# lattice/quda

Hardware: NVIDIA H100
Metric: wilson_dslash_gflops (higher is better)
Workload: dtype f32

## Files before the change

quda_b200/csrc/clover.h:

```cpp
#pragma once

#include "core.h"

namespace b200
{

  template <class P> struct CloverView {
    using store = typename P::store;
    const store *c[2];
    int volume_cb;
    int compressed;
    int dynamic;
    typename P::real diagonal;
    float nrm;
  };

  template <class P> struct CholT { using type = double; };
  template <> struct CholT<PrecH16> { using type = float; };

  template <class P, int CB> B2_HD void clover_load_block(typename P::real *a, const CloverView<P> &A, int x_cb, int parity, int chi)
  {
    using real = typename P::real;
    using V = typename P::svec;
    constexpr int N = P::Ns;
    constexpr int M = (CB + N - 1) / N;
    constexpr int Moff = CB / N;
    real tmp[M * N];
    const V *base = reinterpret_cast<const V *>(A.c[parity]);
#pragma unroll
    for (int i = 0; i < M; i++) {
      const V w = ld<Cache::STREAM>(base + (size_t)(chi * Moff + i) * A.volume_cb + x_cb);
      vec_to_real(tmp + i * N, w);
      if constexpr (P::fixed) {
#pragma unroll
        for (int j = 0; j < N; j++) tmp[i * N + j] *= A.nrm;
      }
    }
    const int sh = (chi * CB) % N;
    if constexpr (CB == 36) {
#pragma unroll
      for (int i = 0; i < 36; i++) a[i] = tmp[i + sh];
    } else {
#pragma unroll
      for (int i = 0; i < 4; i++) a[i] = tmp[i + sh];
#pragma unroll
      for (int i = 6; i < 30; i++) a[i] = tmp[i - 2 + sh];
#pragma unroll
      for (int i = 0; i < 3; i++) {
        const real dev = a[i];
        a[i + 3] = A.diagonal - dev;
        a[i] = A.diagonal + dev;
      }
      a[30] = -a[6];
      a[31] = -a[7];
      a[32] = -a[8];
      a[33] = -a[9];
      a[34] = -a[16];
      a[35] = -a[17];
    }
  }

  B2_HD constexpr int tri_idx(int i, int j) { return 6 + 2 * (15 - (6 - j) * (5 - j) / 2 + i - j - 1); }

  template <typename real> B2_HD void hmat_mul(real *y, const real *a, const real *x)
  {
#pragma unroll
    for (int i = 0; i < 6; i++) {
      real re = a[i] * x[2 * i], im = a[i] * x[2 * i + 1];
#pragma unroll
      for (int j = 0; j < 6; j++) {
        if (j == i) continue;
        const int k = (j < i) ? tri_idx(i, j) : tri_idx(j, i);
        const real ar = a[k];
        const real ai = (j < i) ? a[k + 1] : -a[k + 1];
        re += ar * x[2 * j];
        re -= ai * x[2 * j + 1];
        im += ar * x[2 * j + 1];
        im += ai * x[2 * j];
      }
      y[2 * i] = re;
      y[2 * i + 1] = im;
    }
  }

  template <typename T, typename real> B2_HD void hmat_solve(real *x, const real *a)
  {
    T Lr[6][6], Li[6][6];
#pragma unroll
    for (int i = 0; i < 6; i++) {
#pragma unroll
      for (int j = 0; j < 6; j++) {
        if (j > i) continue;
        T sr = 0, si = 0;
#pragma unroll
        for (int k = 0; k < 6; k++) {
          if (k >= j) continue;
          sr += Lr[i][k] * Lr[j][k];
          sr += Li[i][k] * Li[j][k];
          si += Li[i][k] * Lr[j][k];
          si -= Lr[i][k] * Li[j][k];
        }
        if (i == j) {
          const T d = (T)a[i] - sr;
#if defined(__CUDA_ARCH__)
          Lr[i][i] = (sizeof(T) == 8) ? (T)::rsqrt((double)d) : (T)::rsqrtf((float)d);
#else
          Lr[i][i] = (T)1 / std::sqrt(d);
#endif
          Li[i][i] = 0;
        } else {
          const int k = tri_idx(i, j);
          Lr[i][j] = ((T)a[k] - sr) * Lr[j][j];
          Li[i][j] = ((T)a[k + 1] - si) * Lr[j][j];
        }
      }
    }
    T yr[6], yi[6];
#pragma unroll
    for (int i = 0; i < 6; i++) {
      T r = x[2 * i], m = x[2 * i + 1];
#pragma unroll
      for (int j = 0; j < 6; j++) {
        if (j >= i) continue;
        r -= Lr[i][j] * yr[j];
        r += Li[i][j] * yi[j];
        m -= Lr[i][j] * yi[j];
        m -= Li[i][j] * yr[j];
      }
      yr[i] = r * Lr[i][i];
      yi[i] = m * Lr[i][i];
    }
#pragma unroll
    for (int i = 5; i >= 0; i--) {
      T r = yr[i], m = yi[i];
#pragma unroll
      for (int j = 0; j < 6; j++) {
        if (j <= i) continue;
        r -= Lr[j][i] * yr[j];
        r -= Li[j][i] * yi[j];
        m -= Lr[j][i] * yi[j];
        m += Li[j][i] * yr[j];
      }
      yr[i] = r * Lr[i][i];
      yi[i] = m * Lr[i][i];
    }
#pragma unroll
    for (int i = 0; i < 6; i++) {
      x[2 * i] = (real)yr[i];
      x[2 * i + 1] = (real)yi[i];
    }
  }

  template <class P, bool inverse> B2_HD void clover_apply_site(typename P::real *v, const CloverView<P> &A, int x_cb, int parity)
  {
    using real = typename P::real;
    real r[24];
#pragma unroll
    for (int c = 0; c < 3; c++) {
#pragma unroll
      for (int z = 0; z < 2; z++) {
        const real v0 = v[(0 * 3 + c) * 2 + z], v1 = v[(1 * 3 + c) * 2 + z];
        const real v2 = v[(2 * 3 + c) * 2 + z], v3 = v[(3 * 3 + c) * 2 + z];
        r[(0 * 3 + c) * 2 + z] = -v1 - v3;
        r[(1 * 3 + c) * 2 + z] = v2 + v0;
        r[(2 * 3 + c) * 2 + z] = v3 - v1;
        r[(3 * 3 + c) * 2 + z] = v0 - v2;
      }
    }
#pragma unroll
    for (int chi = 0; chi < 2; chi++) {
      real a[36];
      if (A.compressed)
        clover_load_block<P, 28>(a, A, x_cb, parity, chi);
      else
        clover_load_block<P, 36>(a, A, x_cb, parity, chi);
      if (inverse && A.dynamic) {
        hmat_solve<typename CholT<P>::type>(r + 12 * chi, a);
#pragma unroll
        for (int i = 0; i < 12; i++) r[12 * chi + i] *= (real)0.25;
      } else {
        real y[12];
        hmat_mul(y, a, r + 12 * chi);
#pragma unroll
        for (int i = 0; i < 12; i++) r[12 * chi + i] = y[i];
      }
    }
#pragma unroll
    for (int c = 0; c < 3; c++) {
#pragma unroll
      for (int z = 0; z < 2; z++) {
        const real r0 = r[(0 * 3 + c) * 2 + z], r1 = r[(1 * 3 + c) * 2 + z];
        const real r2 = r[(2 * 3 + c) * 2 + z], r3 = r[(3 * 3 + c) * 2 + z];
        v[(0 * 3 + c) * 2 + z] = r1 + r3;
        v[(1 * 3 + c) * 2 + z] = -r2 - r0;
        v[(2 * 3 + c) * 2 + z] = -r3 + r1;
        v[(3 * 3 + c) * 2 + z] = -r0 + r2;
      }
    }
  }

}
```

quda_b200/csrc/core.h:

```cpp
#pragma once

#include <cmath>
#include <cstddef>
#include <cstdint>
#include <cstring>
#include <type_traits>
#include <utility>

#if defined(__CUDACC__)
#define B2_HD __host__ __device__ __forceinline__
#define B2_D __device__ __forceinline__
#else
#define B2_HD inline
#define B2_D inline
#endif

namespace b200
{

  struct alignas(16) f4 { float x, y, z, w; };
  struct alignas(16) d2 { double x, y; };
  struct alignas(8) f2 { float x, y; };
  struct alignas(16) s8 { short v[8]; };
  struct alignas(8) s4 { short v[4]; };
// ... 371 lines not shown
      }
#pragma unroll
      for (int i = 0; i < 24 / N; i++) {
        V o;
        store *e = reinterpret_cast<store *>(&o);
#pragma unroll
        for (int j = 0; j < N; j++) {
          if constexpr (P::fixed)
            e[j] = f2s(t[i * N + j]);
          else
            e[j] = t[i * N + j];
        }
        st_stream(base + (size_t)i * stride + x_cb, o);
      }
    }
  };

  template <class P> struct GhostView {
    using store = typename P::store;
    store *v;
    float *norm;
    int face_cb;

    B2_HD void load(typename P::real *out, int idx) const
    {
      using V = typename P::ghost_vec;
      constexpr int N = P::Ng;
      const V *base = reinterpret_cast<const V *>(v);
#pragma unroll
      for (int i = 0; i < 12 / N; i++) {
        const V t = ld<Cache::COHERENT>(base + (size_t)i * face_cb + idx);
        vec_to_real(out + i * N, t);
      }
      if constexpr (P::fixed) {
        const float n = ld<Cache::COHERENT>(norm + idx);
#pragma unroll
        for (int i = 0; i < 12; i++) out[i] *= n;
      }
    }

    B2_HD void save(const typename P::real *in, int idx) const
    {
      using V = typename P::ghost_vec;
      constexpr int N = P::Ng;
      V *base = reinterpret_cast<V *>(v);
      typename P::real t[12];
#pragma unroll
      for (int i = 0; i < 12; i++) t[i] = in[i];
      if constexpr (P::fixed) {
        float mx = 0.0f;
#pragma unroll
        for (int i = 0; i < 12; i++) mx = fmaxf(mx, fabsf(t[i]));
        norm[idx] = mx * kFixedInvMax;
        const float sinv = fast_div(kFixedMax, mx);
#pragma unroll
        for (int i = 0; i < 12; i++) t[i] *= sinv;
      }
#pragma unroll
      for (int i = 0; i < 12 / N; i++) {
        V o;
        store *e = reinterpret_cast<store *>(&o);
#pragma unroll
        for (int j = 0; j < N; j++) {
          if constexpr (P::fixed)
            e[j] = f2s(t[i * N + j]);
          else
            e[j] = t[i * N + j];
        }
        base[(size_t)i * face_cb + idx] = o;
      }
    }
  };

  struct GaugeMeta {
    double anisotropy;
    double link_max;
    int t_boundary;
    int first_time_slice;
    int last_time_slice;
    int t_bound_cb;
    int volume_cb;
  };

  template <class P, int recon> struct GaugeView {
    using real = typename P::real;
    using store = typename P::store;
    using V = typename GaugeVec<P, recon>::vec;
    static constexpr int N = GaugeVec<P, recon>::N;
    static constexpr int M = recon / N;

    const store *g[2];
    int stride;
    real aniso, tb, link_scale;
    int t_bound_cb, volume_cb, first_ts, last_ts;

    B2_HD void init(const void *base, size_t parity_offset_bytes, int stride_, const GaugeMeta &m)
    {
      g[0] = reinterpret_cast<const store *>(base);
      g[1] = reinterpret_cast<const store *>(reinterpret_cast<const char *>(base) + parity_offset_bytes);
      stride = stride_;
      aniso = (real)m.anisotropy;
      tb = (real)m.t_boundary;
      link_scale = (real)m.link_max;
      t_bound_cb = m.t_bound_cb;
      volume_cb = m.volume_cb;
      first_ts = m.first_time_slice;
      last_ts = m.last_time_slice;
    }

    B2_HD real u0(int dir, int idx) const
    {
      if (dir < 3) return aniso;
      if (idx >= volume_cb) return first_ts ? tb : (real)1;
      if (idx >= t_bound_cb) return last_ts ? tb : (real)1;
      return (real)1;
    }

    struct Raw {
      V w[M];
    };

    template <Cache c = Cache::STREAM> B2_HD void load_raw(Raw &r, int dir, int x_cb, int parity) const
    {
      const V *base = reinterpret_cast<const V *>(g[parity]);
#pragma unroll
      for (int i = 0; i < M; i++) r.w[i] = ld<c>(base + (size_t)(dir * M + i) * stride + x_cb);
    }

    B2_HD void unpack(real *u, const Raw &r, int dir, int x_cb) const
    {
      real t[recon];
#pragma unroll
      for (int i = 0; i < M; i++) {
        vec_to_real(t + i * N, r.w[i]);
        if constexpr (P::fixed) {
#pragma unroll
          for (int j = 0; j < N; j++) t[i * N + j] *= kFixedInvMax;
        }
      }
      if constexpr (recon == 18) {
#pragma unroll
        for (int i = 0; i < 18; i++) u[i] = P::fixed ? link_scale * t[i] : t[i];
      } else if constexpr (recon == 12) {
#pragma unroll
        for (int i = 0; i < 12; i++) u[i] = t[i];
        const real s = u0(dir, x_cb);
        const cplx<real> a0 {u[0], u[1]}, a1 {u[2], u[3]}, a2 {u[4], u[5]};
        const cplx<real> b0 {u[6], u[7]}, b1 {u[8], u[9]}, b2 {u[10], u[11]};
        cplx<real> c0 = cmul(a1, b2), c1 = cmul(a2, b0), c2 = cmul(a0, b1);
        const cplx<real> d0 = cmul(a2, b1), d1 = cmul(a0, b2), d2_ = cmul(a1, b0);
        u[12] = s * (c0.re - d0.re);
        u[13] = -s * (c0.im - d0.im);
        u[14] = s * (c1.re - d1.re);
        u[15] = -s * (c1.im - d1.im);
        u[16] = s * (c2.re - d2_.re);
        u[17] = -s * (c2.im - d2_.im);
      } else {
        unpack8(u, t, u0(dir, x_cb));
      }
    }

    B2_HD void unpack_deferred(real *u, real &scale, const Raw &r, int dir, int x_cb) const
    {
      static_assert(P::fixed, "deferred scaling is for the fixed-point formats");
      if constexpr (recon == 8) {
        unpack(u, r, dir, x_cb);
        scale = (real)1;
      } else {
        real t[recon];
        vecs_to_real<M, N>(t, r.w);
        if constexpr (recon == 18) {
#pragma unroll
          for (int i = 0; i < 18; i++) u[i] = t[i];
          scale = link_scale * kFixedInvMax;
        } else {
#pragma unroll
          for (int i = 0; i < 12; i++) u[i] = t[i];
          const real s = u0(dir, x_cb) * kFixedInvMax;
          const cplx<real> a0 {u[0], u[1]}, a1 {u[2], u[3]}, a2 {u[4], u[5]};
          const cplx<real> b0 {u[6], u[7]}, b1 {u[8], u[9]}, b2 {u[10], u[11]};
          cplx<real> c0 = cmul(a1, b2), c1 = cmul(a2, b0), c2 = cmul(a0, b1);
          const cplx<real> d0 = cmul(a2, b1), d1 = cmul(a0, b2), d2_ = cmul(a1, b0);
          u[12] = s * (c0.re - d0.re);
          u[13] = -s * (c0.im - d0.im);
          u[14] = s * (c1.re - d1.re);
          u[15] = -s * (c1.im - d1.im);
          u[16] = s * (c2.re - d2_.re);
          u[17] = -s * (c2.im - d2_.im);
          scale = kFixedInvMax;
        }
      }
    }

    template <Cache c = Cache::STREAM> B2_HD void load(real *u, int dir, int x_cb, int parity) const
    {
      Raw r;
      load_raw<c>(r, dir, x_cb, parity);
      unpack(u, r, dir, x_cb);
    }

    B2_HD static void unpack8(real *u, const real *in, real u0v)
    {
      const real u0_inv = rcp_((real)u0v);
      cplx<real> o[9];
      o[1] = {in[2], in[3]};
      o[2] = {in[4], in[5]};
      o[3] = {in[6], in[7]};
      real sn, cs;
      sincospi_(in[0], &sn, &cs);
      o[0] = {cs, sn};
      sincospi_(in[1], &sn, &cs);
      o[6] = {cs, sn};
      real row_sum = mul_rn(o[1].re, o[1].re);
      row_sum = fma_rn(o[1].im, o[1].im, row_sum);
      row_sum = fma_rn(o[2].re, o[2].re, row_sum);
      row_sum = fma_rn(o[2].im, o[2].im, row_sum);
      const real row_sum_inv = rcp_(row_sum);
      real diff = fma_rn(u0_inv, u0_inv, -row_sum);
      const real m00 = diff > 0 ? diff * rsqrt_(diff) : (real)0;
      o[0].re *= m00;
      o[0].im *= m00;
      real col_sum = mul_rn(o[0].re, o[0].re);
      col_sum = fma_rn(o[0].im, o[0].im, col_sum);
      col_sum = fma_rn(o[3].re, o[3].re, col_sum);
      col_sum = fma_rn(o[3].im, o[3].im, col_sum);
      diff = fma_rn(u0_inv, u0_inv, -col_sum);
      const real m20 = diff > 0 ? diff * rsqrt_(diff) : (real)0;
      o[6].re *= m20;
      o[6].im *= m20;
      const real r_inv2 = u0_inv * row_sum_inv;
      {
        cplx<real> A = cmul(conj(o[0]), o[3]);
        A.re *= u0v;
        A.im *= u0v;
        cplx<real> t4 = cmul(conj(o[6]), conj(o[2]));
        const cplx<real> a1 = cmul(A, o[1]);
        o[4] = {-r_inv2 * (t4.re + a1.re), -r_inv2 * (t4.im + a1.im)};
        cplx<real> t5 = cmul(conj(o[6]), conj(o[1]));
        const cplx<real> a2 = cmul(A, o[2]);
        o[5] = {r_inv2 * (t5.re - a2.re), r_inv2 * (t5.im - a2.im)};
      }
      {
        cplx<real> A = cmul(conj(o[0]), o[6]);
        A.re *= u0v;
        A.im *= u0v;
        cplx<real> t7 = cmul(conj(o[3]), conj(o[2]));
        const cplx<real> a1 = cmul(A, o[1]);
        o[7] = {r_inv2 * (t7.re - a1.re), r_inv2 * (t7.im - a1.im)};
        cplx<real> t8 = cmul(conj(o[3]), conj(o[1]));
        const cplx<real> a2 = cmul(A, o[2]);
        o[8] = {-r_inv2 * (t8.re + a2.re), -r_inv2 * (t8.im + a2.im)};
      }
#pragma unroll
      for (int i = 0; i < 3; i++) {
        u[2 * i] = o[i + 3].re;
        u[2 * i + 1] = o[i + 3].im;
        u[6 + 2 * i] = o[i].re;
        u[6 + 2 * i + 1] = o[i].im;
        u[12 + 2 * i] = -o[i + 6].re;
        u[12 + 2 * i + 1] = -o[i + 6].im;
      }
    }

    B2_HD static float rcp_(float x)
    {
#if defined(__CUDA_ARCH__)
      return __frcp_rn(x);
#else
      return 1.0f / x;
#endif
    }
    B2_HD static double rcp_(double x) { return 1.0 / x; }
    B2_HD static void sincospi_(float x, float *s, float *c)
    {
#if defined(__CUDA_ARCH__)
      __sincosf(x * 3.14159265358979323846f, s, c);
#else
      *s = (float)std::sin(3.14159265358979323846 * (double)x);
      *c = (float)std::cos(3.14159265358979323846 * (double)x);
#endif
    }
    B2_HD static void sincospi_(double x, double *s, double *c)
    {
#if defined(__CUDA_ARCH__)
      ::sincospi(x, s, c);
#else
      *s = std::sin(3.14159265358979323846 * x);
      *c = std::cos(3.14159265358979323846 * x);
#endif
    }
    B2_HD static float rsqrt_(float x)
    {
#if defined(__CUDA_ARCH__)
      return ::rsqrtf(x);
#else
      return 1.0f / std::sqrt(x);
#endif
    }
    B2_HD static double rsqrt_(double x)
    {
#if defined(__CUDA_ARCH__)
      return ::rsqrt(x);
#else
      return 1.0 / std::sqrt(x);
#endif
    }
  };

  template <bool adjoint, typename real> B2_HD void su3_mul(real *r, const real *u, const real *h)
  {
#pragma unroll
    for (int s = 0; s < 2; s++) {
#pragma unroll
      for (int i = 0; i < 3; i++) {
        real re = 0, im = 0;
#pragma unroll
        for (int j = 0; j < 3; j++) {
          const real ur = adjoint ? u[(j * 3 + i) * 2] : u[(i * 3 + j) * 2];
          const real ui = adjoint ? -u[(j * 3 + i) * 2 + 1] : u[(i * 3 + j) * 2 + 1];
          const real hr = h[(s * 3 + j) * 2], hi = h[(s * 3 + j) * 2 + 1];
          re = fma_rn(ur, hr, re);
          re = fma_rn(-ui, hi, re);
          im = fma_rn(ur, hi, im);
          im = fma_rn(ui, hr, im);
        }
        r[(s * 3 + i) * 2] = re;
        r[(s * 3 + i) * 2 + 1] = im;
      }
    }
  }

  template <typename real> B2_HD void project(real *h, const real *v, int mu, int sign)
  {
    const real sg = (real)sign;
#pragma unroll
    for (int c = 0; c < 3; c++) {
      const real v0r = v[(0 * 3 + c) * 2], v0i = v[(0 * 3 + c) * 2 + 1];
      const real v1r = v[(1 * 3 + c) * 2], v1i = v[(1 * 3 + c) * 2 + 1];
      const real v2r = v[(2 * 3 + c) * 2], v2i = v[(2 * 3 + c) * 2 + 1];
      const real v3r = v[(3 * 3 + c) * 2], v3i = v[(3 * 3 + c) * 2 + 1];
      real h0r, h0i, h1r, h1i;
      if (mu == 0) {
        h0r = v0r - sg * v3i;
        h0i = v0i + sg * v3r;
        h1r = v1r - sg * v2i;
        h1i = v1i + sg * v2r;
      } else if (mu == 1) {
        h0r = v0r + sg * v3r;
        h0i = v0i + sg * v3i;
        h1r = v1r - sg * v2r;
        h1i = v1i - sg * v2i;
      } else if (mu == 2) {
        h0r = v0r - sg * v2i;
        h0i = v0i + sg * v2r;
        h1r = v1r + sg * v3i;
// ... 83 lines not shown
```

quda_b200/csrc/kernels.cuh:

```cuda
#pragma once

#include <cstdlib>
#include <cuda_runtime.h>

#include "dslash_site.h"
#include "plan.h"

namespace b200
{

#ifndef B2_MINBLOCKS_F64
#define B2_MINBLOCKS_F64 2
#endif
#ifndef B2_MINBLOCKS_F32
#define B2_MINBLOCKS_F32 4
#endif
#ifndef B2_MINBLOCKS_H16
#define B2_MINBLOCKS_H16 4
#endif
  template <class P> struct MinBlocks { static constexpr int value = B2_MINBLOCKS_F32; };
  template <> struct MinBlocks<PrecF64> { static constexpr int value = B2_MINBLOCKS_F64; };
  template <> struct MinBlocks<PrecH16> { static constexpr int value = B2_MINBLOCKS_H16; };

#ifndef B2_L2_PREFETCH
#define B2_L2_PREFETCH 0
#endif
  __device__ __forceinline__ void prefetch_l2(const void *p) { asm volatile("prefetch.global.L2 [%0];" ::"l"(p)); }

  template <class P, int recon>
  __device__ __forceinline__ void prefetch_future_tile(const DslashArgs<P, recon> &arg, const TileMap &tm)
  {
    using GV = GaugeView<P, recon>;
    constexpr int lanes_per_line = 128 / sizeof(typename GV::V);
    if ((threadIdx.x & ((1 << tm.sh[0]) - 1)) % lanes_per_line != 0) return;
    const unsigned gx = gridDim.x, gy = gridDim.y, gz = gridDim.z;
    unsigned lin = blockIdx.x + gx * (blockIdx.y + gy * blockIdx.z) + B2_L2_PREFETCH;
    if (lin >= gx * gy * gz) return;
    const unsigned bz = lin / (gx * gy);
    lin -= bz * gx * gy;
    const unsigned by = lin / gx;
    const unsigned bx = lin - by * gx;
    int x[4], x_cb, parity;
    if (!tile_site(x, x_cb, parity, arg.geom, tm, arg.n_parity, arg.parity, bx, by, bz, threadIdx.x)) return;
    const Geom &g = arg.geom;
    const typename GV::V *gf = reinterpret_cast<const typename GV::V *>(arg.U.g[parity]);
    const typename GV::V *gb = reinterpret_cast<const typename GV::V *>(arg.U.g[1 - parity]);
#pragma unroll
    for (int d = 0; d < 4; d++) {
      int y[4] = {x[0], x[1], x[2], x[3]};
      y[d] = (x[d] - 1 < 0) ? g.X[d] - 1 : x[d] - 1;
      const int n_cb = cb_from_coords(y, g);
#pragma unroll
      for (int i = 0; i < GV::M; i++) {
        prefetch_l2(gf + (size_t)(d * GV::M + i) * arg.U.stride + x_cb);
        prefetch_l2(gb + (size_t)(d * GV::M + i) * arg.U.stride + n_cb);
      }
    }
  }

  template <class P, int recon, bool dagger, bool xpay, OpType op, bool part>
  __global__ void __launch_bounds__(kMaxTile, MinBlocks<P>::value)
    dslash_interior_kernel(const __grid_constant__ DslashArgs<P, recon> arg, const __grid_constant__ TileMap tm)
  {
    if constexpr (B2_L2_PREFETCH > 0) prefetch_future_tile(arg, tm);
    int x[4], x_cb, parity;
    if (!tile_site(x, x_cb, parity, arg.geom, tm, arg.n_parity, arg.parity, blockIdx.x, blockIdx.y, blockIdx.z, threadIdx.x))
      return;
    dslash_site_interior<P, recon, dagger, xpay, op, part>(arg, x, x_cb, parity);
  }

  __device__ __forceinline__ unsigned ld_acquire_sys(const unsigned *p)
  {
    unsigned v;
    asm volatile("ld.acquire.sys.global.u32 %0, [%1];" : "=r"(v) : "l"(p) : "memory");
    return v;
  }
  __device__ __forceinline__ void st_release_sys(unsigned *p, unsigned v)
  {
    asm volatile("st.release.sys.global.u32 [%0], %1;" ::"l"(p), "r"(v) : "memory");
  }
  __device__ __forceinline__ void red_release_sys_add(unsigned *p, unsigned v)
  {
    asm volatile("red.release.sys.global.add.u32 [%0], %1;" ::"l"(p), "r"(v) : "memory");
  }

  template <class Arg> __device__ __forceinline__ void wait_for_halo(const Arg &arg)
  {
    if (threadIdx.x == 0) {
      const long long t0 = clock64();
      const unsigned uses = (arg.seq + (arg.seq & 1u)) >> 1;
#pragma unroll
      for (int d = 0; d < 4; d++) {
#pragma unroll
        for (int dir = 0; dir < 2; dir++) {
          const unsigned *f = arg.wait_flag[d][dir];
          if (!f) continue;
          const unsigned target = uses * (unsigned)arg.geom.face_cb[d];
          while ((int)(ld_acquire_sys(f) - target) < 0) {
            if (clock64() - t0 > 20000000000LL) {
              if (arg.timeout_flag) *arg.timeout_flag = 1;
              break;
            }
            __nanosleep(100);
          }
        }
      }
    }
    __syncthreads();
  }

  template <class P, int recon, bool dagger, bool xpay, OpType op>
  __global__ void __launch_bounds__(kMaxTile, MinBlocks<P>::value)
    dslash_boundary_kernel(const __grid_constant__ DslashArgs<P, recon> arg, const __grid_constant__ TileMap tm,
                           const __grid_constant__ SlabTable st)
  {
    wait_for_halo(arg);
    const int parity = arg.n_parity == 2 ? blockIdx.y : arg.parity;
    int x[4], x_cb;
    if (!slab_site(x, x_cb, arg.geom, tm, st, parity, blockIdx.x, threadIdx.x)) return;
    dslash_site_full<P, recon, dagger, xpay, op>(arg, x, x_cb, parity);
  }

  template <class P, int recon, bool dagger, bool xpay, OpType op>
  __global__ void __launch_bounds__(256) dslash_exterior_kernel(const __grid_constant__ DslashArgs<P, recon> arg)
  {
    wait_for_halo(arg);
    const int parity = arg.n_parity == 2 ? blockIdx.y : arg.parity;
    const int tid = blockIdx.x * blockDim.x + threadIdx.x;
    if (tid >= arg.threads_ext[4]) return;
    int x[4], x_cb;
    if (!exterior_thread_site(x, x_cb, arg, tid, parity)) return;
    dslash_site_exterior<P, recon, dagger, xpay, op>(arg, x, x_cb, parity);
  }

  template <class P, bool inverse>
  __global__ void __launch_bounds__(256) clover_apply_kernel(SpinorView<P> out, SpinorView<P> in, CloverView<P> A,
                                                             int volume_cb, int parity)
  {
    const int x_cb = blockIdx.x * blockDim.x + threadIdx.x;
    if (x_cb >= volume_cb) return;
    typename P::real v[24];
    in.template load<Cache::COHERENT>(v, x_cb);
    clover_apply_site<P, inverse>(v, A, x_cb, parity);
    out.save(v, x_cb);
  }

// ... 244 lines not shown
    count_launch();
    return check_cuda(cudaGetLastError(), "copy_gauge launch");
  }

  template <class P> int launch_gauge_copy_precision(const GaugeCopyRequest &rq)
  {
    const bool dbl = rq.host_precision == 8;
    switch (rq.native.reconstruct) {
    case 18: return dbl ? launch_gauge_copy_typed<P, 18, double>(rq) : launch_gauge_copy_typed<P, 18, float>(rq);
    case 12: return dbl ? launch_gauge_copy_typed<P, 12, double>(rq) : launch_gauge_copy_typed<P, 12, float>(rq);
    case 8: return dbl ? launch_gauge_copy_typed<P, 8, double>(rq) : launch_gauge_copy_typed<P, 8, float>(rq);
    }
    return set_error(B200_ERR_INVALID, "reconstruct %d not in {18,12,8}", rq.native.reconstruct);
  }

  template <class P, typename H>
  __global__ void __launch_bounds__(128) copy_clover_kernel(typename P::store *c0, typename P::store *c1, const H *packed,
                                                            int volume_cb, int compressed, double diagonal, double nrm_inv)
  {
    using store = typename P::store;
    constexpr int N = P::Ns;
    const int x = blockIdx.x * blockDim.x + threadIdx.x;
    if (x >= volume_cb) return;
    const int parity = blockIdx.y;
    store *dst = parity ? c1 : c0;
    const H *src = packed + ((size_t)parity * volume_cb + x) * 72;
    const int CB = compressed ? 28 : 36;
#pragma unroll
    for (int chi = 0; chi < 2; chi++) {
      double a[36];
#pragma unroll
      for (int i = 0; i < 36; i++) a[i] = 0.5 * (double)src[chi * 36 + i];
      for (int k = 0; k < CB; k++) {
        double v;
        if (!compressed)
          v = a[k];
        else if (k < 3)
          v = a[k] - diagonal;
        else if (k == 3)
          v = 0.0;
        else
          v = a[k + 2];
        const int flat = chi * CB + k;
        store o;
        if constexpr (P::fixed)
          o = f2s((float)(v * nrm_inv));
        else
          o = (store)v;
        dst[((size_t)(flat / N) * volume_cb + x) * N + flat % N] = o;
      }
    }
  }

  template <class P> int launch_clover_copy_precision(const CloverCopyRequest &rq)
  {
    Geom g;
    geom_init(g, rq.X);
    auto *c0 = reinterpret_cast<typename P::store *>(const_cast<void *>(rq.native.clover));
    auto *c1 = reinterpret_cast<typename P::store *>(reinterpret_cast<char *>(const_cast<void *>(rq.native.clover)) + rq.native.parity_stride_bytes);
    const double nrm_inv = P::fixed ? (2.0 * 32767.0) / rq.native.max_element : 1.0;
    dim3 grid((g.volume_cb + 127) / 128, 2, 1);
    cudaStream_t s = (cudaStream_t)rq.stream;
    if (rq.host_precision == 8)
      copy_clover_kernel<P, double><<<grid, 128, 0, s>>>(c0, c1, (const double *)rq.packed, g.volume_cb, rq.native.compressed, rq.native.diagonal, nrm_inv);
    else
      copy_clover_kernel<P, float><<<grid, 128, 0, s>>>(c0, c1, (const float *)rq.packed, g.volume_cb, rq.native.compressed, rq.native.diagonal, nrm_inv);
    count_launch();
    return check_cuda(cudaGetLastError(), "copy_clover launch");
  }

  template <class P, int recon, bool dagger, bool xpay, OpType op>
  int launch_config(OpCfg<dagger, xpay, op>, const LaunchRequest &rq, const DslashArgs<P, recon> &arg)
  {
    LaunchPlan pl;
    if (int rc = plan_dslash(pl, rq, arg)) return rc;
    cudaStream_t s = (cudaStream_t)rq.stream;
    for (int i = 0; i < pl.n; i++) {
      const LaunchStep &l = pl.step[i];
      const dim3 grid(l.grid[0], l.grid[1], l.grid[2]);
      switch (l.kind) {
      case LAUNCH_INTERIOR:
        if (l.masked)
          dslash_interior_kernel<P, recon, dagger, xpay, op, true><<<grid, l.threads, 0, s>>>(arg, l.tm);
        else
          dslash_interior_kernel<P, recon, dagger, xpay, op, false><<<grid, l.threads, 0, s>>>(arg, l.tm);
        break;
      case LAUNCH_BOUNDARY: dslash_boundary_kernel<P, recon, dagger, xpay, op><<<grid, l.threads, 0, s>>>(arg, l.tm, l.st); break;
      case LAUNCH_EXTERIOR: dslash_exterior_kernel<P, recon, dagger, xpay, op><<<grid, l.threads, 0, s>>>(arg); break;
      case LAUNCH_FUSED: {
        PackArgs<P> pk {};
        if (rq.fused_pack) fill_pack_args(pk, *rq.fused_pack);
        dslash_fused_kernel<P, recon, dagger, xpay, op><<<grid, l.threads, 0, s>>>(arg, l.tm, pk, l.fs);
        break;
      }
      }
      count_launch();
    }
    return check_cuda(cudaGetLastError(), rq.fused_pack ? "fused dslash launch" : "dslash launch");
  }

  template <class P> int launch_precision(const LaunchRequest &rq)
  {
    return dispatch_dslash<P>(rq, [&](auto c, const auto &arg) { return launch_config(c, rq, arg); });
  }

  template <class P> int launch_clover_precision(const CloverRequest &rq)
  {
    SpinorView<P> out, in;
    CloverView<P> A;
    fill_spinor(out, rq.out, rq.out_norm, rq.volume_cb);
    fill_spinor(in, rq.in, rq.in_norm, rq.volume_cb);
    fill_clover(A, rq.A, rq.volume_cb);
    const int blocks = (rq.volume_cb + 127) / 128;
    cudaStream_t s = (cudaStream_t)rq.stream;
    if (rq.inverse)
      clover_apply_kernel<P, true><<<blocks, 128, 0, s>>>(out, in, A, rq.volume_cb, rq.parity);
    else
      clover_apply_kernel<P, false><<<blocks, 128, 0, s>>>(out, in, A, rq.volume_cb, rq.parity);
    count_launch();
    return check_cuda(cudaGetLastError(), "clover launch");
  }

  template <class P> int launch_twist_precision(const TwistRequest &rq)
  {
    SpinorView<P> out, in;
    fill_spinor(out, rq.out, rq.out_norm, rq.volume_cb);
    fill_spinor(in, rq.in, rq.in_norm, rq.volume_cb);
    twist_gamma5_kernel<P><<<(rq.volume_cb + 255) / 256, 256, 0, (cudaStream_t)rq.stream>>>(out, in, rq.volume_cb, (typename P::real)rq.a,
                                                                                          (typename P::real)rq.b);
    count_launch();
    return check_cuda(cudaGetLastError(), "twist launch");
  }

  template <class P> int launch_pack_precision(const PackRequest &rq)
  {
    int gx;
    if (int rc = pack_blocks(gx, rq)) return rc;
    if (!gx) return 0;
    PackArgs<P> arg;
    fill_pack_args(arg, rq);
    pack_kernel<P><<<dim3(gx, 8, 1), 128, 0, (cudaStream_t)rq.stream>>>(arg);
    count_launch();
    return check_cuda(cudaGetLastError(), "pack launch");
  }

  template <class P> int launch_pack_multi_precision(const PackRequest &rq, const PackBatchRequest &b)
  {
    int gx;
    if (int rc = pack_blocks(gx, rq)) return rc;
    if (!gx) return 0;
    PackArgs<P> arg;
    fill_pack_args(arg, rq);
    PackBatch<P> batch;
    fill_pack_batch(batch, b, arg.geom.volume_cb);
    pack_multi_kernel<P><<<dim3(gx, 8, b.n_src), 128, 0, (cudaStream_t)rq.stream>>>(arg, batch);
    count_launch();
    return check_cuda(cudaGetLastError(), "batched pack launch");
  }

}
```

quda_b200/csrc/launch.h:

```cpp
#pragma once

#include <cstdarg>
#include <cstdio>
#include <cuda_runtime.h>

#include "../../include/b200_dslash.h"
#include "dslash_site.h"

namespace b200
{

  int set_error(int code, const char *fmt, ...);
  int check_cuda(cudaError_t e, const char *what);
  void count_launch();

  struct LaunchRequest {
    int op, kernel, reconstruct, dagger, xpay, parity, n_parity;
    int X[4], tile[4];
    double b;
    int asymmetric;
    int tma;
    int tma_ty, tma_tz, tma_grid;
    int tma_link_slots;
    int tma_center_slots, tma_halo_slots;
// ... 39 lines not shown
    int volume_cb, host_precision, to_native;
    void *stream;
  };

  struct GaugeCopyRequest {
    b200_gauge native;
    int X[4];
    void *qdp[4], *ghost[4];
    int host_precision;
    void *stream;
  };

  struct CloverCopyRequest {
    b200_clover native;
    int X[4];
    const void *packed;
    int host_precision;
    void *stream;
  };

  struct PackRequest {
    int X[4], parity, dagger, comm_dim[4];
    void *in, *in_norm;
    void *dst[4][2], *dst_norm[4][2];
    void *signal[4][2];
    int *block_counter;
    unsigned seq;
    void *stream;
  };

  inline size_t ghost_parity_bytes(int precision, const int X[4], int dim)
  {
    const size_t face_cb = (size_t)X[0] * X[1] * X[2] * X[3] / X[dim] / 2;
    return face_cb * (12 * (size_t)precision + (precision == B200_HALF ? 4 : 0));
  }

  inline int check_src_stride(const char *what, int n_src, int precision, const int X[4], const int comm_dim[4], const size_t stride[4],
                              int n_parity)
  {
    for (int d = 0; d < 4; d++) {
      if (!comm_dim[d] || n_src <= 1) continue;
      const size_t slab = (size_t)n_parity * ghost_parity_bytes(precision, X, d);
      if (stride[d] < slab)
        return set_error(B200_ERR_INVALID, "%s[%d] = %zu is smaller than one face (%zu bytes): every source needs its own ghost slab", what, d,
                         stride[d], slab);
      if (stride[d] % 16) return set_error(B200_ERR_INVALID, "%s[%d] = %zu is not a multiple of 16 bytes", what, d, stride[d]);
    }
    return 0;
  }

  struct PackBatchRequest {
    int n_src;
    void *in[B200_MAX_MULTI_RHS], *in_norm[B200_MAX_MULTI_RHS];
    size_t dst_stride[4];
  };

  template <class P> void fill_spinor(SpinorView<P> &v, void *base, void *norm, int volume_cb)
  {
    v.v = reinterpret_cast<typename P::store *>(base);
    v.stride = volume_cb;
    if (P::fixed)
      v.norm = norm ? reinterpret_cast<float *>(norm) :
                      reinterpret_cast<float *>(reinterpret_cast<short *>(base) + (size_t)24 * volume_cb);
    else
      v.norm = nullptr;
  }

  template <class P> void fill_spinor_parity(SpinorView<P> &v, const b200_spinor &f, int p)
  {
    char *base = reinterpret_cast<char *>(f.v) + (size_t)p * f.parity_stride_bytes;
    char *norm = f.norm ? reinterpret_cast<char *>(f.norm) + (size_t)p * f.parity_stride_bytes : nullptr;
    fill_spinor(v, base, norm, f.volume_cb);
  }

  template <class P> void fill_clover(CloverView<P> &A, const b200_clover &c, int volume_cb)
  {
    A.c[0] = reinterpret_cast<const typename P::store *>(c.clover);
    A.c[1] = reinterpret_cast<const typename P::store *>(reinterpret_cast<const char *>(c.clover) + c.parity_stride_bytes);
    A.volume_cb = volume_cb;
    A.compressed = c.compressed;
    A.dynamic = c.dynamic_inverse;
    A.diagonal = (typename P::real)c.diagonal;
    A.nrm = (float)(c.max_element / (2.0 * 32767.0));
  }

  template <class P> void fill_ghost(GhostView<P> &g, void *base, void *norm, int face_cb)
  {
    g.v = reinterpret_cast<typename P::store *>(base);
    g.face_cb = face_cb;
    if (P::fixed)
      g.norm = norm ? reinterpret_cast<float *>(norm) :
                      (base ? reinterpret_cast<float *>(reinterpret_cast<short *>(base) + (size_t)12 * face_cb) : nullptr);
    else
      g.norm = nullptr;
  }

  template <class P> B2_HD GhostView<P> ghost_of_source(GhostView<P> g, size_t bytes)
  {
    g.v = reinterpret_cast<typename P::store *>(reinterpret_cast<char *>(g.v) + bytes);
    if (g.norm) g.norm = reinterpret_cast<float *>(reinterpret_cast<char *>(g.norm) + bytes);
    return g;
  }

  template <class P, int recon> int fill_args(DslashArgs<P, recon> &arg, const LaunchRequest &rq)
  {
    geom_init(arg.geom, rq.X);
    const Geom &g = arg.geom;
    arg.n_parity = rq.n_parity;
    arg.parity = rq.parity;
    arg.a = (typename P::real)rq.a;
    arg.A = CloverView<P> {};
    arg.A.diagonal = (typename P::real)(rq.dagger ? -rq.b : rq.b);
    if (rq.out.volume_cb != g.volume_cb || rq.in.volume_cb != g.volume_cb)
      return set_error(B200_ERR_INVALID, "spinor volume_cb (%d/%d) does not match lattice (%d)", rq.out.volume_cb,
                       rq.in.volume_cb, g.volume_cb);
    if (rq.n_parity == 2) {
      for (int p = 0; p < 2; p++) {
        fill_spinor_parity(arg.out[p], rq.out, p);
        fill_spinor_parity(arg.in[p], rq.in, p);
        if (rq.xpay) fill_spinor_parity(arg.x[p], rq.x, p);
      }
    } else {
      fill_spinor_parity(arg.out[rq.parity], rq.out, 0);
      fill_spinor_parity(arg.in[1 - rq.parity], rq.in, 0);
      if (rq.xpay) fill_spinor_parity(arg.x[rq.parity], rq.x, 0);
    }
    GaugeMeta m;
    m.anisotropy = rq.U.anisotropy;
    m.link_max = rq.U.link_max;
    m.t_boundary = rq.U.t_boundary;
    m.first_time_slice = rq.U.first_time_slice;
    m.last_time_slice = rq.U.last_time_slice;
    m.t_bound_cb = (g.X[3] - 1) * g.X[0] * g.X[1] * g.X[2] / 2;
    m.volume_cb = g.volume_cb;
    arg.U.init(rq.U.gauge, rq.U.parity_stride_bytes, rq.U.stride, m);
    if (rq.op == OP_CLOVER || rq.op == OP_CLOVER_PC) fill_clover(arg.A, rq.A, g.volume_cb);
    arg.threads_ext[0] = 0;
    for (int d = 0; d < 4; d++) {
      arg.comm_dim[d] = rq.halo.comm_dim[d] ? 1 : 0;
      if (arg.comm_dim[d] && g.X[d] < 4)
        return set_error(B200_ERR_INVALID, "partitioned dimension %d needs local extent >= 4 (got %d)", d, g.X[d]);
      arg.threads_ext[d + 1] = arg.threads_ext[d] + (arg.comm_dim[d] ? 2 * g.face_cb[d] : 0);
      const size_t parity_elems = (size_t)12 * g.face_cb[d] + (P::fixed ? 2 * g.face_cb[d] : 0);
      arg.ghost_parity_stride[d] = rq.n_parity == 2 ? parity_elems : 0;
      arg.ghost_norm_parity_stride[d] = rq.n_parity == 2 ? parity_elems / 2 : 0;
      for (int dir = 0; dir < 2; dir++) {
        if (arg.comm_dim[d] && rq.kernel != B200_KERNEL_INTERIOR && rq.kernel != B200_KERNEL_INTERIOR_TILES
            && rq.kernel != B200_KERNEL_INTERIOR_SITES && !rq.halo.ghost[d][dir])
          return set_error(B200_ERR_INVALID, "dimension %d is partitioned but halo.ghost[%d][%d] is NULL", d, d, dir);
        fill_ghost(arg.ghost[d][dir], rq.halo.ghost[d][dir], rq.halo.ghost_norm[d][dir], g.face_cb[d]);
        arg.wait_flag[d][dir] = arg.comm_dim[d] ? reinterpret_cast<const unsigned *>(rq.halo.wait_flag[d][dir]) : nullptr;
      }
    }
    arg.seq = rq.halo.seq;
    arg.timeout_flag = rq.halo.timeout_flag;
    return 0;
  }


  template <class P> int mrhs_batch(int remaining, int max_batch)
  {
    int cap = sizeof(typename P::real) == 8 ? 2 : 4;
    if (max_batch > 0 && max_batch < cap) cap = max_batch;
    if (remaining >= 4 && cap >= 4) return 4;
    if (remaining >= 2 && cap >= 2) return 2;
    return 1;
// ... 306 lines not shown
```

Baseline: 6387.

## Defer fixed-point clover scaling, specialize float Cholesky, speed recon-8 unpack, add PDL launch

For half-precision clover, the per-element dequantization multiply is dropped and the scale is applied once on output, with a quantized diagonal and inverse scale precomputed on the host. A float specialization of the Cholesky solve uses FMAs and a reciprocal-diagonal array. Recon-8 gauge unpacking for fixed precision folds the pi scale into fast sincos, uses a precomputed inverse anisotropy, and uses an approximate reciprocal with a Newton step. The unmasked interior kernel is now launched with programmatic dependent launch so it can overlap the previous kernel's tail. The fixed-point changes do not apply to f32, and fast sincos and the approximate reciprocal lower accuracy in the half path.

New measurement: 6498 (median of 6 runs). No clear change (+1.7%).

```diff
diff --git a/quda_b200/csrc/clover.h b/quda_b200/csrc/clover.h
--- a/quda_b200/csrc/clover.h
+++ b/quda_b200/csrc/clover.h
@@ -5,7 +5,13 @@
 namespace b200
 {
 
-  template <class P> struct CloverView {
+  template <class P> struct CloverFixedScale {};
+  template <> struct CloverFixedScale<PrecH16> {
+    float diagonal_q;
+    float inv_scale;
+  };
+
+  template <class P> struct CloverView : CloverFixedScale<P> {
     using store = typename P::store;
     const store *c[2];
     int volume_cb;
@@ -31,10 +37,6 @@
     for (int i = 0; i < M; i++) {
       const V w = ld<Cache::STREAM>(base + (size_t)(chi * Moff + i) * A.volume_cb + x_cb);
       vec_to_real(tmp + i * N, w);
-      if constexpr (P::fixed) {
-#pragma unroll
-        for (int j = 0; j < N; j++) tmp[i * N + j] *= A.nrm;
-      }
     }
     const int sh = (chi * CB) % N;
     if constexpr (CB == 36) {
@@ -45,11 +47,16 @@
       for (int i = 0; i < 4; i++) a[i] = tmp[i + sh];
 #pragma unroll
       for (int i = 6; i < 30; i++) a[i] = tmp[i - 2 + sh];
+      real diag;
+      if constexpr (P::fixed)
+        diag = A.diagonal_q;
+      else
+        diag = A.diagonal;
 #pragma unroll
       for (int i = 0; i < 3; i++) {
         const real dev = a[i];
-        a[i + 3] = A.diagonal - dev;
-        a[i] = A.diagonal + dev;
+        a[i + 3] = diag - dev;
+        a[i] = diag + dev;
       }
       a[30] = -a[6];
       a[31] = -a[7];
@@ -151,6 +158,79 @@
     }
   }
 
+  template <> B2_HD void hmat_solve<float, float>(float *x, const float *a)
+  {
+    float Lr[6][6], Li[6][6], dinv[6];
+#pragma unroll
+    for (int i = 0; i < 6; i++) {
+#pragma unroll
+      for (int j = 0; j < 6; j++) {
+        if (j > i) continue;
+        if (i == j) {
+          float d = a[i];
+#pragma unroll
+          for (int k = 0; k < 6; k++) {
+            if (k >= j) continue;
+            d = fma_rn(-Lr[i][k], Lr[i][k], d);
+            d = fma_rn(-Li[i][k], Li[i][k], d);
+          }
+#if defined(__CUDA_ARCH__)
+          dinv[i] = ::rsqrtf(d);
+#else
+          dinv[i] = 1.0f / std::sqrt(d);
+#endif
+        } else {
+          const int t = tri_idx(i, j);
+          float sr = a[t], si = a[t + 1];
+#pragma unroll
+          for (int k = 0; k < 6; k++) {
+            if (k >= j) continue;
+            sr = fma_rn(-Lr[i][k], Lr[j][k], sr);
+            sr = fma_rn(-Li[i][k], Li[j][k], sr);
+            si = fma_rn(-Li[i][k], Lr[j][k], si);
+            si = fma_rn(Lr[i][k], Li[j][k], si);
+          }
+          Lr[i][j] = mul_rn(sr, dinv[j]);
+          Li[i][j] = mul_rn(si, dinv[j]);
+        }
+      }
+    }
+    float yr[6], yi[6];
+#pragma unroll
+    for (int i = 0; i < 6; i++) {
+      float r = x[2 * i], m = x[2 * i + 1];
+#pragma unroll
+      for (int j = 0; j < 6; j++) {
+        if (j >= i) continue;
+        r = fma_rn(-Lr[i][j], yr[j], r);
+        r = fma_rn(Li[i][j], yi[j], r);
+        m = fma_rn(-Lr[i][j], yi[j], m);
+        m = fma_rn(-Li[i][j], yr[j], m);
+      }
+      yr[i] = mul_rn(r, dinv[i]);
+      yi[i] = mul_rn(m, dinv[i]);
+    }
+#pragma unroll
+    for (int i = 5; i >= 0; i--) {
+      float r = yr[i], m = yi[i];
+#pragma unroll
+      for (int j = 0; j < 6; j++) {
+        if (j <= i) continue;
+        r = fma_rn(-Lr[j][i], yr[j], r);
+        r = fma_rn(-Li[j][i], yi[j], r);
+        m = fma_rn(-Lr[j][i], yi[j], m);
+        m = fma_rn(Li[j][i], yr[j], m);
+      }
+      yr[i] = mul_rn(r, dinv[i]);
+      yi[i] = mul_rn(m, dinv[i]);
+    }
+#pragma unroll
+    for (int i = 0; i < 6; i++) {
+      x[2 * i] = yr[i];
+      x[2 * i + 1] = yi[i];
+    }
+  }
+
   template <class P, bool inverse> B2_HD void clover_apply_site(typename P::real *v, const CloverView<P> &A, int x_cb, int parity)
   {
     using real = typename P::real;
@@ -176,14 +256,32 @@
         clover_load_block<P, 36>(a, A, x_cb, parity, chi);
       if (inverse && A.dynamic) {
         hmat_solve<typename CholT<P>::type>(r + 12 * chi, a);
-#pragma unroll
-        for (int i = 0; i < 12; i++) r[12 * chi + i] *= (real)0.25;
+        if constexpr (!P::fixed) {
+#pragma unroll
+          for (int i = 0; i < 12; i++) r[12 * chi + i] *= (real)0.25;
+        }
       } else {
         real y[12];
         hmat_mul(y, a, r + 12 * chi);
 #pragma unroll
         for (int i = 0; i < 12; i++) r[12 * chi + i] = y[i];
       }
+    }
+    if constexpr (P::fixed) {
+      const real s = (inverse && A.dynamic) ? A.inv_scale : A.nrm;
+#pragma unroll
+      for (int c = 0; c < 3; c++) {
+#pragma unroll
+        for (int z = 0; z < 2; z++) {
+          const real r0 = r[(0 * 3 + c) * 2 + z], r1 = r[(1 * 3 + c) * 2 + z];
+          const real r2 = r[(2 * 3 + c) * 2 + z], r3 = r[(3 * 3 + c) * 2 + z];
+          v[(0 * 3 + c) * 2 + z] = s * (r1 + r3);
+          v[(1 * 3 + c) * 2 + z] = -s * (r2 + r0);
+          v[(2 * 3 + c) * 2 + z] = s * (r1 - r3);
+          v[(3 * 3 + c) * 2 + z] = s * (r2 - r0);
+        }
+      }
+      return;
     }
 #pragma unroll
     for (int c = 0; c < 3; c++) {
diff --git a/quda_b200/csrc/core.h b/quda_b200/csrc/core.h
--- a/quda_b200/csrc/core.h
+++ b/quda_b200/csrc/core.h
@@ -477,7 +477,12 @@
     int volume_cb;
   };
 
-  template <class P, int recon> struct GaugeView {
+  template <class P, int recon> struct GaugeRecon8Consts {};
+  template <> struct GaugeRecon8Consts<PrecH16, 8> {
+    float aniso_inv;
+  };
+
+  template <class P, int recon> struct GaugeView : GaugeRecon8Consts<P, recon> {
     using real = typename P::real;
     using store = typename P::store;
     using V = typename GaugeVec<P, recon>::vec;
@@ -501,6 +506,7 @@
       volume_cb = m.volume_cb;
       first_ts = m.first_time_slice;
       last_ts = m.last_time_slice;
+      if constexpr (P::fixed && recon == 8) this->aniso_inv = (real)(1.0 / m.anisotropy);
     }
 
     B2_HD real u0(int dir, int idx) const
@@ -530,7 +536,8 @@
         vec_to_real(t + i * N, r.w[i]);
         if constexpr (P::fixed) {
 #pragma unroll
-          for (int j = 0; j < N; j++) t[i * N + j] *= kFixedInvMax;
+          for (int j = 0; j < N; j++)
+            if (recon != 8 || i * N + j >= 2) t[i * N + j] *= kFixedInvMax;
         }
       }
       if constexpr (recon == 18) {
@@ -550,8 +557,12 @@
         u[15] = -s * (c1.im - d1.im);
         u[16] = s * (c2.re - d2_.re);
         u[17] = -s * (c2.im - d2_.im);
+      } else if constexpr (P::fixed) {
+        const real u0v = u0(dir, x_cb);
+        unpack8(u, t, u0v, dir < 3 ? this->aniso_inv : u0v);
       } else {
-        unpack8(u, t, u0(dir, x_cb));
+        const real u0v = u0(dir, x_cb);
+        unpack8(u, t, u0v, rcp_(u0v));
       }
     }
 
@@ -594,23 +605,29 @@
       unpack(u, r, dir, x_cb);
     }
 
-    B2_HD static void unpack8(real *u, const real *in, real u0v)
-    {
-      const real u0_inv = rcp_((real)u0v);
+    B2_HD static void unpack8(real *u, const real *in, real u0v, real u0_inv)
+    {
       cplx<real> o[9];
       o[1] = {in[2], in[3]};
       o[2] = {in[4], in[5]};
       o[3] = {in[6], in[7]};
       real sn, cs;
-      sincospi_(in[0], &sn, &cs);
-      o[0] = {cs, sn};
-      sincospi_(in[1], &sn, &cs);
-      o[6] = {cs, sn};
+      if constexpr (P::fixed) {
+        sincos_(in[0] * (real)(3.14159265358979323846 * kFixedInvMax), &sn, &cs);
+        o[0] = {cs, sn};
+        sincos_(in[1] * (real)(3.14159265358979323846 * kFixedInvMax), &sn, &cs);
+        o[6] = {cs, sn};
+      } else {
+        sincospi_(in[0], &sn, &cs);
+        o[0] = {cs, sn};
+        sincospi_(in[1], &sn, &cs);
+        o[6] = {cs, sn};
+      }
       real row_sum = mul_rn(o[1].re, o[1].re);
       row_sum = fma_rn(o[1].im, o[1].im, row_sum);
       row_sum = fma_rn(o[2].re, o[2].re, row_sum);
       row_sum = fma_rn(o[2].im, o[2].im, row_sum);
-      const real row_sum_inv = rcp_(row_sum);
+      const real row_sum_inv = P::fixed ? rcp_nr(row_sum) : rcp_(row_sum);
       real diff = fma_rn(u0_inv, u0_inv, -row_sum);
       const real m00 = diff > 0 ? diff * rsqrt_(diff) : (real)0;
       o[0].re *= m00;
@@ -666,6 +683,25 @@
 #endif
     }
     B2_HD static double rcp_(double x) { return 1.0 / x; }
+    B2_HD static float rcp_nr(float x)
+    {
+#if defined(__CUDA_ARCH__)
+      float r;
+      asm("rcp.approx.ftz.f32 %0, %1;" : "=f"(r) : "f"(x));
+      return fma_rn(r, fma_rn(-x, r, 1.0f), r);
+#else
+      return 1.0f / x;
+#endif
+    }
+    B2_HD static void sincos_(float x, float *s, float *c)
+    {
+#if defined(__CUDA_ARCH__)
+      __sincosf(x, s, c);
+#else
+      *s = (float)std::sin((double)x);
+      *c = (float)std::cos((double)x);
+#endif
+    }
     B2_HD static void sincospi_(float x, float *s, float *c)
     {
 #if defined(__CUDA_ARCH__)
diff --git a/quda_b200/csrc/kernels.cuh b/quda_b200/csrc/kernels.cuh
--- a/quda_b200/csrc/kernels.cuh
+++ b/quda_b200/csrc/kernels.cuh
@@ -62,6 +62,10 @@
   __global__ void __launch_bounds__(kMaxTile, MinBlocks<P>::value)
     dslash_interior_kernel(const __grid_constant__ DslashArgs<P, recon> arg, const __grid_constant__ TileMap tm)
   {
+    if constexpr (!part) {
+      asm volatile("griddepcontrol.launch_dependents;" ::: "memory");
+      asm volatile("griddepcontrol.wait;" ::: "memory");
+    }
     if constexpr (B2_L2_PREFETCH > 0) prefetch_future_tile(arg, tm);
     int x[4], x_cb, parity;
     if (!tile_site(x, x_cb, parity, arg.geom, tm, arg.n_parity, arg.parity, blockIdx.x, blockIdx.y, blockIdx.z, threadIdx.x))
@@ -472,8 +476,19 @@
       case LAUNCH_INTERIOR:
         if (l.masked)
           dslash_interior_kernel<P, recon, dagger, xpay, op, true><<<grid, l.threads, 0, s>>>(arg, l.tm);
-        else
-          dslash_interior_kernel<P, recon, dagger, xpay, op, false><<<grid, l.threads, 0, s>>>(arg, l.tm);
+        else {
+          cudaLaunchConfig_t cfg = {};
+          cfg.gridDim = grid;
+          cfg.blockDim = dim3(l.threads);
+          cfg.stream = s;
+          cudaLaunchAttribute attr[1];
+          attr[0].id = cudaLaunchAttributeProgrammaticStreamSerialization;
+          attr[0].val.programmaticStreamSerializationAllowed = 1;
+          cfg.attrs = attr;
+          cfg.numAttrs = 1;
+          if (cudaError_t e = cudaLaunchKernelEx(&cfg, dslash_interior_kernel<P, recon, dagger, xpay, op, false>, arg, l.tm))
+            return check_cuda(e, "dslash launch");
+        }
         break;
       case LAUNCH_BOUNDARY: dslash_boundary_kernel<P, recon, dagger, xpay, op><<<grid, l.threads, 0, s>>>(arg, l.tm, l.st); break;
       case LAUNCH_EXTERIOR: dslash_exterior_kernel<P, recon, dagger, xpay, op><<<grid, l.threads, 0, s>>>(arg); break;
diff --git a/quda_b200/csrc/launch.h b/quda_b200/csrc/launch.h
--- a/quda_b200/csrc/launch.h
+++ b/quda_b200/csrc/launch.h
@@ -145,6 +145,11 @@
     A.dynamic = c.dynamic_inverse;
     A.diagonal = (typename P::real)c.diagonal;
     A.nrm = (float)(c.max_element / (2.0 * 32767.0));
+    if constexpr (P::fixed) {
+      const double nrm = c.max_element / (2.0 * 32767.0);
+      A.diagonal_q = (float)(c.diagonal / nrm);
+      A.inv_scale = (float)(0.25 / nrm);
+    }
   }
 
   template <class P> void fill_ghost(GhostView<P> &g, void *base, void *norm, int face_cb)
```
